# mmdagent/distantspeechrecognition-mirror

Measured on AMD Instinct MI355X. Metric: decoded_audio_hours_per_sec, higher is better.
Workload: dtype f32

## Files before the change

distantspeechrecognition-mirror_amd/csrc/decoder.cpp:

```cpp
#include "common.h"
#include "wfst_graph.h"
#include "lattice.h"
#include "lexicon.h"
#include "wordtrace.h"
#include "viterbi.h"
#include "decode_plan.h"
#include <algorithm>
#include <cmath>

namespace dsr {

static_assert(kPlanSideBytes == (size_t) kSideLds * sizeof(Side), "decode_plan.h budgets the side records of viterbi.h");

struct DecoderState {
  dsr_decoder_cfg cfg; bool haveGraph = false; int nSlots = 0; int nNodes = 0;
  WfstGraph::Csr csr; WfstGraph::Tables tab;
  DevBuf<int> d_xoff, d_xarc, d_xpathOff, d_eoff, d_path, d_nodeFinal, d_queue; DevBuf<float> d_pathCost;
  DevBuf<XRec> d_xrec; DevBuf<ERec> d_erec; DevBuf<float> d_arcCost, d_nodeCost; DevBuf<uint32_t> d_arcOut, d_arcIn;
  DevBuf<TokA> d_tokA, d_ctok; DevBuf<TokB> d_tokB; DevBuf<Side> d_side; DevBuf<XRecD> d_xrecD; DevBuf<XRecC> d_xrecC; double recLmScale = 0.0;  int fastOK = 0; int maxCnt = 0; DevBuf<int> d_tokOff, d_tokCnt, d_owner, d_rank, d_chead; DevBuf<unsigned> d_tags; DevBuf<CandA> d_cA; DevBuf<CandB> d_cB; DevBuf<unsigned> d_first; DevBuf<Bp> d_arena;
  DevBuf<long long> d_prof; DevBuf<dsr_decode_result> d_res; DevBuf<int> d_arcs; DevBuf<unsigned> d_words;
  long arenaCap = 0; int initial = 0; unsigned tokenMemoryLimit = 0;
  long lastPoolCap = 0;
  hipEvent_t evTrace = nullptr;
  DevBuf<TraceHead> d_heads; DevBuf<int> d_hopRec, d_hopOff;
// ... 363 lines not shown
    if (d->pendingU > 0) throw Error(DSR_E_CONSISTENCY, "a decode is already in flight on this decoder: collect it first");
    if (U <= 0) return;
    hipStream_t st = (hipStream_t) stream;
    if (d->cfg.wordTrace) { launch_wordtrace(d, score, nframes, U, Tmax, nDist, maxPath, want_paths, st); return; }
    check_arc_inputs(d, nDist);
    const bool latOn = d->cfg.latticeTokens > 0;
    if (latOn && d->dumpOn) throw Error(DSR_E_PARAMETER, "lattice bookkeeping and the token dump are separate debugging aids: enable one");
    const VitEnv env = read_vit_env();
    PlanIn in; in.streams = d->cfg.streams; in.maxActive = d->cfg.maxActive; in.arenaTokens = d->cfg.arenaTokens; in.latticeTokens = d->cfg.latticeTokens;
    in.topN = d->cfg.topN; in.dumpOn = d->dumpOn != 0; in.nNodes = d->nNodes; in.maxCnt = d->maxCnt; in.U = U; in.Tmax = Tmax; in.nDist = nDist;
    in.staticLds = viterbi_static_lds(plan_base_modes(in, env));
    const DecodePlan P = plan_decode(in, env, [&] { return xcd_round_robin(st); });
    ensure_scratch(d, P.slots, Tmax, latOn ? U : (P.segFrames > 0 ? P.poolArenas : 0));
    if (maxPath < 0) maxPath = 0;
    const VitArgs A = fill_vit_args(d, P, env, score, nframes, U, Tmax, nDist, maxPath, want_paths != 0, st);
    if (env.segVerbose) fprintf(stderr, "[dsr viterbi] %d utterances on %d workgroups: %s, %s state table\n", U, P.slots, P.segFrames > 0 ? (P.segQueues == 8 ? "time-sliced, XCD-bound queues" : "time-sliced, one queue") : "run to completion", P.narrow ? "narrow" : "wide");
    const TraceArgs TA = fill_trace_args(d, A);
    order_behind_last_traceback(P.slots, st);
    viterbi_launch(P.modes, A, P.slots, P.ldsBytes, st);
    traceback_launch(TA, st);
    publish_traceback(d, st);
    enqueue_result_copies(d, U, want_paths ? (size_t) U * maxPath : 0, st);
    d->pendingSlots = P.slots; d->pendingProf = A.D.prof;
  });
}

static void report_profile(const long long* prof, int slots)
{
  std::vector<long long> hp((size_t) slots * kProfN); DSR_HIP(hipMemcpy(hp.data(), prof, hp.size() * sizeof(long long), hipMemcpyDeviceToHost));
  double acc[32] = {0}; for (int s2 = 0; s2 < slots; s2++) for (int i = 0; i < 32; i++) acc[i] += (double) hp[(size_t) s2 * kProfN + i];
  fprintf(stderr, "[dsr viterbi prof] mean us per slot:");
  for (int i = 0; i < 32; i++) if (i != 15) fprintf(stderr, " p%d=%.0f", i, acc[i] / slots / 100.0);
  fprintf(stderr, "\n");
  double tmin = 1e30, tmax = 0.0, tsum = 0.0;
  for (int s2 = 0; s2 < slots; s2++) { double t = 0.0; for (int i = 0; i < 32; i++) if (i != 15) t += (double) hp[(size_t) s2 * kProfN + i]; t /= 100.0; tsum += t; if (t < tmin) tmin = t; if (t > tmax) tmax = t; }
  {
    double h[12] = {0}; for (int s2 = 0; s2 < slots; s2++) for (int i = 0; i < 12; i++) h[i] += (double) hp[(size_t) s2 * kProfN + 32 + i];
    const double nf = h[0] + h[1] + h[2] + h[3], tk = h[4] + h[5] + h[6] + h[7];
    static const char* const cn[4] = {"<=8192", "<=12288", ">12288", "memory path"};
    for (int c = 0; c < 4; c++) if (h[c] > 0) fprintf(stderr, "[dsr viterbi prof] frames with %s placements: %.1f %% of the frames, %.1f %% of the frame time, %.1f us per frame, %.2f ns per placement\n",
                                                      cn[c], 100.0 * h[c] / nf, 100.0 * h[4 + c] / tk, h[4 + c] / 100.0 / h[c], h[4 + c] * 10.0 / h[8 + c]);
  }
  {
    double a = 0, b = 0; for (int s2 = 0; s2 < slots; s2++) { a += (double) hp[(size_t) s2 * kProfN + 44]; b += (double) hp[(size_t) s2 * kProfN + 45]; }
    if (a + b > 0) fprintf(stderr, "[dsr viterbi prof] register-path frames: %.1f %% start laid out, %.1f %% run P1/P2\n", 100.0 * a / (a + b), 100.0 * b / (a + b));
    double m1 = 0, m2 = 0, mAll = 0; for (int s2 = 0; s2 < slots; s2++) { m1 += (double) hp[(size_t) s2 * kProfN + 46]; m2 += (double) hp[(size_t) s2 * kProfN + 47]; mAll += (double) hp[(size_t) s2 * kProfN + 32 + 3]; }
    if (mAll > 0) fprintf(stderr, "[dsr viterbi prof] memory-path frames: %.0f, of them %.1f %% with at most 28672 placements, %.1f %% with at most 32767\n", mAll, 100.0 * m1 / mAll, 100.0 * m2 / mAll);
  }
  {
    double h[6] = {0}; for (int s2 = 0; s2 < slots; s2++) for (int i = 0; i < 6; i++) h[i] += (double) hp[(size_t) s2 * kProfN + 48 + i];
    if (h[0] > 0) fprintf(stderr, "[dsr viterbi prof] hops behind the first: %.0f wave-placements, %.1f %% with a path of two or more hops, %.1f %% load hop costs, %.1f %% run the hop loop; "
                                  "%.3f hop iterations per wave-placement for %.3f hops per lane (x 64: %.2f)\n",
                          h[0], 100.0 * h[1] / h[0], 100.0 * h[2] / h[0], 100.0 * h[3] / h[0], h[4] / h[0], h[5] / h[0] / 64.0, h[5] / h[0]);
  }
  fprintf(stderr, "[dsr viterbi prof] busy us per slot: mean %.0f min %.0f max %.0f\n", tsum / slots, tmin, tmax);
  if (slots >= 64 && slots % 8 == 0) {
    double bx[8] = {0}; for (int s2 = 0; s2 < slots; s2++) { double t = 0.0; for (int i = 0; i < 32; i++) if (i != 15) t += (double) hp[(size_t) s2 * kProfN + i]; bx[s2 & 7] += t / 100.0; }
    fprintf(stderr, "[dsr viterbi prof] busy us per slot, by XCD:"); for (int q = 0; q < 8; q++) fprintf(stderr, " %.0f", bx[q] / (slots / 8)); fprintf(stderr, "\n");
  }
}

dsr_status dsr_decoder_decode_collect(dsr_decoder* d, dsr_decode_result* res, int32_t* arcs_out, uint32_t* words_out)
{
  return guard([&] {
    if (!d || !res) throw Error(DSR_E_PARAMETER, "null argument");
    if (d->pendingU <= 0) throw Error(DSR_E_CONSISTENCY, "no decode in flight");
    const int U = d->pendingU; const size_t nPath = d->pendingPath; const int slots = d->pendingSlots; long long* prof = d->pendingProf;
    d->pendingU = 0; d->lastU = U; d->lastPaths = nPath > 0; d->lastMaxPath = nPath > 0 ? nPath / (size_t) U : 0;
    DSR_HIP(hipEventSynchronize(d->evDone));
    memcpy(res, d->h_res.p, sizeof(dsr_decode_result) * U);
    if (arcs_out && nPath) memcpy(arcs_out, d->h_arcs.p, sizeof(int) * nPath);
    if (words_out && nPath) memcpy(words_out, d->h_words.p, sizeof(unsigned) * nPath);
    if (read_vit_env().segVerbose && d->d_poolNext.p && d->lastPoolCap > 0) {
      unsigned long long used = 0; DSR_HIP(hipMemcpy(&used, d->d_poolNext.p, sizeof(used), hipMemcpyDeviceToHost));
      fprintf(stderr, "[dsr viterbi] pool of back-pointer records: %.1f M of %.1f M taken\n", used / 1e6, d->lastPoolCap / 1e6);
    }
    if (read_vit_env().segVerbose) {
      long long laid = 0, reg = 0, all = 0;
      for (int u = 0; u < U; u++) if (res[u].status == DSR_OK || res[u].status == DSR_E_DIMENSION) { laid += res[u].laidOutFrames_; reg += res[u].registerFrames; all += res[u].frames + 1; }
      fprintf(stderr, "[dsr viterbi] frames: %lld laid out by the frame before, %lld through P1/P2, %lld on the memory path\n", laid, reg - laid, all - reg);
    }
    if (prof) report_profile(prof, slots);
    if (d->dumpOn) {
      long cnt[2]; DSR_HIP(hipMemcpy(cnt, d->d_dumpCount.p, sizeof(cnt), hipMemcpyDeviceToHost));
      const long N = cnt[0] < d->dumpCap ? cnt[0] : d->dumpCap; d->h_dumpFrames = cnt[1];
      std::vector<long> fo(cnt[1] + 1); if (cnt[1] > 0) DSR_HIP(hipMemcpy(fo.data(), d->d_dumpFrameOff.p, sizeof(long) * (cnt[1] + 1), hipMemcpyDeviceToHost));
      d->h_dumpFrameOff.assign(fo.begin(), fo.end());
      d->h_dumpNode.resize(N); d->h_dumpArc.resize(N); d->h_dumpAc.resize(N); d->h_dumpLm.resize(N);
      if (N > 0) {
        DSR_HIP(hipMemcpy(d->h_dumpNode.data(), d->d_dumpNode.p, sizeof(int) * N, hipMemcpyDeviceToHost));
        DSR_HIP(hipMemcpy(d->h_dumpArc.data(), d->d_dumpArc.p, sizeof(int) * N, hipMemcpyDeviceToHost));
        DSR_HIP(hipMemcpy(d->h_dumpAc.data(), d->d_dumpAc.p, sizeof(float) * N, hipMemcpyDeviceToHost));
        DSR_HIP(hipMemcpy(d->h_dumpLm.data(), d->d_dumpLm.p, sizeof(float) * N, hipMemcpyDeviceToHost));
      }
    }
  });
}

dsr_status dsr_decoder_decode_batch(dsr_decoder* d, const float* score, const int32_t* nframes, int U, int Tmax, int nDist,
                                    dsr_decode_result* res, int32_t* arcs_out, uint32_t* words_out, int maxPath, void* stream)
{
  if (!res) return guard([&] { throw Error(DSR_E_PARAMETER, "null argument"); });
  if (U <= 0) return DSR_OK;
  const dsr_status s1 = dsr_decoder_decode_launch(d, score, nframes, U, Tmax, nDist, maxPath, (arcs_out || words_out) ? 1 : 0, stream);
  if (s1 != DSR_OK) return s1;
  return dsr_decoder_decode_collect(d, res, arcs_out, words_out);
// ... 118 lines not shown
```

distantspeechrecognition-mirror_amd/csrc/k_viterbi.hip:

```cpp
#include "launch.h"
#include "viterbi.h"
#include <algorithm>
#include <cmath>
#include <type_traits>

namespace dsr {

static constexpr uint32_t kNone = 0xFFFFFFFFu;
static constexpr uint32_t kEndBit = 0x80000000u;
static constexpr int kWaves = kThreads / 64;
static constexpr int kFastK = 8;
static constexpr int kB = 2;
static constexpr int kFastE = 8190;
static constexpr int kP1 = 16;
static constexpr int kW = 4;

typedef const __attribute__((address_space(4))) VitArgs* KP;

__device__ __forceinline__ unsigned ld_u32(const unsigned* p) { return __hip_atomic_load(p, __ATOMIC_RELAXED, __HIP_MEMORY_SCOPE_AGENT); }
__device__ __forceinline__ int ld_i32(const int* p) { return __hip_atomic_load(p, __ATOMIC_RELAXED, __HIP_MEMORY_SCOPE_AGENT); }
__device__ __forceinline__ void st_u32(unsigned* p, unsigned v) { __hip_atomic_store(p, v, __ATOMIC_RELAXED, __HIP_MEMORY_SCOPE_AGENT); }
__device__ __forceinline__ void st_i32(int* p, int v) { __hip_atomic_store(p, v, __ATOMIC_RELAXED, __HIP_MEMORY_SCOPE_AGENT); }
__device__ __forceinline__ void st_u64_dev(void* p, unsigned long long v) { __hip_atomic_store(reinterpret_cast<unsigned long long*>(p), v, __ATOMIC_RELAXED, __HIP_MEMORY_SCOPE_AGENT); }
__device__ __forceinline__ unsigned long long ld_u64_dev(const void* p) { return __hip_atomic_load(reinterpret_cast<const unsigned long long*>(p), __ATOMIC_RELAXED, __HIP_MEMORY_SCOPE_AGENT); }

__device__ __forceinline__ int wave_incl_scan(int v, int )
{
  v += __builtin_amdgcn_update_dpp(0, v, 0x111, 0xF, 0xF, true);
  v += __builtin_amdgcn_update_dpp(0, v, 0x112, 0xF, 0xF, true);
  v += __builtin_amdgcn_update_dpp(0, v, 0x114, 0xF, 0xF, true);
  v += __builtin_amdgcn_update_dpp(0, v, 0x118, 0xF, 0xF, true);
  v += __builtin_amdgcn_update_dpp(0, v, 0x142, 0xA, 0xF, false);
  v += __builtin_amdgcn_update_dpp(0, v, 0x143, 0xC, 0xF, false);
  return v;
}
__device__ __forceinline__ float wave_max_f_uni(float v)
{
#define DSR_DPP_F(ctrl, rm) { const float o = __int_as_float(__builtin_amdgcn_update_dpp(__float_as_int(v), __float_as_int(v), ctrl, rm, 0xF, false)); v = fmaxf(v, o); }
  DSR_DPP_F(0x111, 0xF) DSR_DPP_F(0x112, 0xF) DSR_DPP_F(0x114, 0xF) DSR_DPP_F(0x118, 0xF) DSR_DPP_F(0x142, 0xA) DSR_DPP_F(0x143, 0xC)
#undef DSR_DPP_F
  return __int_as_float(__builtin_amdgcn_readlane(__float_as_int(v), 63));
}
__device__ __forceinline__ double wave_min_d_uni(double v)
{
#define DSR_DPP_D(ctrl, rm) { const int lo = __double2loint(v), hi = __double2hiint(v); \
    const double o = __hiloint2double(__builtin_amdgcn_update_dpp(hi, hi, ctrl, rm, 0xF, false), __builtin_amdgcn_update_dpp(lo, lo, ctrl, rm, 0xF, false)); v = (o < v) ? o : v; }
  DSR_DPP_D(0x111, 0xF) DSR_DPP_D(0x112, 0xF) DSR_DPP_D(0x114, 0xF) DSR_DPP_D(0x118, 0xF) DSR_DPP_D(0x142, 0xA) DSR_DPP_D(0x143, 0xC)
#undef DSR_DPP_D
  return __hiloint2double(__builtin_amdgcn_readlane(__double2hiint(v), 63), __builtin_amdgcn_readlane(__double2loint(v), 63));
}
__device__ __forceinline__ double wave_min_d(double v)
{
#pragma unroll
  for (int d = 32; d >= 1; d >>= 1) { const double o = __shfl_xor(v, d, 64); v = (o < v) ? o : v; }
// ... 244 lines not shown
            }
          }
          TICK(16);
          for (int i = tid; i < kFastC / 32; i += nthr) s_bm[i] = 0u;
          TICK(17);
#pragma unroll
          for (int it = 0; it < kP1; it++) {
            const int base = b0 + it * 64; pk[it] = 0u;
            if (base < b1) {
              const int i = base + lane; int cnt = 0;
              if (i < b1) {
                if (!((double) psc[it] > thresh)) cnt = pcn[it];
              }
              pcn[it] = cnt;
              const int incl = wave_incl_scan(cnt, lane);
              const unsigned long long bal = __ballot(cnt > 0);
              if (cnt > 0) pk[it] = 0x80000000u | (unsigned) ((runC + incl - cnt) & 0x7FFF) | ((unsigned) ((runE + __popcll(bal & ((1ull << lane) - 1ull))) & 0xFFFF) << 15);
              runC += __builtin_amdgcn_readlane(incl, 63); runE += __popcll(bal);
            }
          }
          TICK(18);
          if (lane == 0) { s_waveTot[wave] = runC; s_waveTotE[wave] = runE; }
          if (tid == 0) { s_sideN = 0; s_gbase[0] = 0; s_err = 0; }
        }
        __syncthreads();
        TICK(0);
        int cbase, ebase;
        {
          const int a = (lane < nw) ? s_waveTot[lane] : 0, b = (lane < nw) ? s_waveTotE[lane] : 0;
          const int sa = wave_incl_scan(a, lane), sb = wave_incl_scan(b, lane);
          C = __builtin_amdgcn_readlane(sa, 63); E = __builtin_amdgcn_readlane(sb, 63);
          const int wu = uni(wave);
          cbase = __builtin_amdgcn_readlane(sa - a, wu); ebase = __builtin_amdgcn_readlane(sb - b, wu);
        }
        TICK(19);
        if (!(C > fastCapC || E > eCap || C > regC)) {
          RELOAD();
          const bool ident = (E == n);
#pragma unroll
          for (int it = 0; it < kP1; it++) if (pk[it] & 0x80000000u) {
            const int e = ebase + (int) ((pk[it] >> 15) & 0xFFFFu); const int off = cbase + (int) (pk[it] & 0x7FFFu);
            if (!ident) ctok[e] = curA[wave * chunkT + it * 64 + lane];
            atomicOr(&s_bm[off >> 5], 1u << (off & 31));
            for (int g = (off >> 6) + 1; g <= ((off + pcn[it]) >> 6); g++) s_gbase[g] = (unsigned) (e + 1) | ((unsigned) (64 * g - off) << 13);
          }
          __syncthreads();
        }
        } else __syncthreads();
        if (C > fastCapC || E > eCap || C > regC) { fast = false; __syncthreads(); }
        else {
          RELOAD();
          const bool ident = (E == n);
          const TokA* __restrict__ ctk = ident ? curA : ctok;
          TICK(1);
          Cfr = C;
          if (pre && tid == nthr - 1) s_stat[2] += 1ll << 32;
          if (PROF && tid == 0) s_hist[pre ? 12 : 13] += 1;
          RELOAD();
          int tq = tid; asm volatile("" : "+v"(tq)); const int lq = tq & 63, wq = tq >> 6;
          const int K = (C + nthr - 1) / nthr;
          float qac[kFastK], qlm[kFastK]; int qrec[kFastK]; unsigned ek[kFastK];
          double* const ttlS = reinterpret_cast<double*>(cA);
          uint4* const ovf = reinterpret_cast<uint4*>(cB);
          const XRecD* const xrecD = ka->G.xrecD; const float* const pathCost = ka->G.pathCost; const uint32_t silenceX = ka->D.silenceX;
          double locMin = HUGE_VAL; float locMag = 0.0f;
          const bool prevNull0 = (fr == 0);
          const double lmS = ka->D.lmScale, lsPen = __dmul_rn(ka->D.lmScale, ka->D.lmPenalty), lsSil = __dmul_rn(ka->D.lmScale, ka->D.silPenalty);
          const bool sil0 = (0u == silenceX);
#pragma unroll
          for (int k = 0; k < kFastK; k++) { qac[k] = 0.0f; qlm[k] = 0.0f; qrec[k] = 0; ek[k] = 0u; }

          const int nPass = (!NARROW && C > tableC) ? 2 : 1;
          auto table_insert = [&](const unsigned dst, const unsigned prod, const int c) __attribute__((always_inline)) -> unsigned {
            const unsigned key = dst + 1u;
            unsigned h = (prod >> 7) & (unsigned) (tabN - 1); int probes = 0;
            if (NARROW) {
              const unsigned w = (key << 15) | (unsigned) c;
              for (;;) {
                const unsigned kk = atomicCAS(&tab[h], 0u, w);
                if (kk == 0u) break;
                if ((kk >> 15) == key) { atomicMin(&tab[h], w); break; }
                h = (h + 1u) & (unsigned) (tabN - 1);
                if (++probes > tabN) { s_err = 1; break; }
              }
              return h;
            }
            for (;;) {
              const unsigned kk = atomicCAS(&hkey[h], 0u, key);
              if (kk == 0u || kk == key) break;
              h = (h + 1u) & (unsigned) (hashN - 1);
              if (++probes > hashN) { s_err = 1; break; }
            }
            atomicMin(&hfirst[h], (unsigned) c);
            return h;
          };
          constexpr unsigned ekBucket = NARROW ? 0x7FFFu : 0x3FFFu;
          auto in_pass = [&](const unsigned e, const int pass) __attribute__((always_inline)) -> bool { return NARROW || (int) ((e >> 27) & 1u) == pass; };
          auto is_first = [&](const unsigned h, const int c) __attribute__((always_inline)) -> bool { return NARROW ? (tab[h] & 0x7FFFu) == (unsigned) c : hfirst[h] == (unsigned) c; };
          auto push_side = [&](const unsigned h, const int sx) __attribute__((always_inline)) -> unsigned {
            if (NARROW) {
              unsigned old = tab[h];
              for (;;) { const unsigned prev = atomicCAS(&tab[h], old, 0x80000000u | ((unsigned) sx << 15) | (old & 0x7FFFu)); if (prev == old) break; old = prev; }
              return (old & 0x80000000u) ? (0x80000000u | ((old >> 15) & 0xFFFFu)) : 0u;
            }
            return atomicExch(&hkey[h], 0x80000000u | (unsigned) sx);
          };
// ... 63 lines not shown
#pragma unroll
              for (int h = 1; h < 4; h++) {
                double l = __dadd_rn((double) lmNode, __dmul_rn(lmS, (double) hc[i][h - 1]));
                if (!NP) { const double l1 = __dadd_rn(l, lsPen); l = ((xmeta >> (17 + h)) & 1u) ? l1 : l; }
                lmNode = (pls[i] > h) ? (float) l : lmNode;
              }
              if (PROF) TICK(31);
              lm8[i] = lmNode;
            }
            bool anyMore = false;
#pragma unroll
            for (int i = 0; i < kB; i++) anyMore = anyMore || more[i];
            if (__any(anyMore)) {
#pragma unroll
              for (int i = 0; i < kB; i++) if (more[i]) {
                const uint32_t xmeta = (uint32_t) xr[i].y; const int plen = (int) (xmeta & 0xFFFFu), xp2 = xr[i].w;
                double lmNode = (double) lm8[i];
                if (!(xmeta & 0x80000000u)) {
                  for (int h = 4; h < plen; h++) {
                    double l = __dadd_rn(lmNode, __dmul_rn(lmS, (double) pathCost[xp2 + h - 1]));
                    if (!NP && ((xmeta >> (17 + h)) & 1u)) l = __dadd_rn(l, lsPen);
                    lmNode = (double) (float) l;
                  }
                } else {
                  const int* pp = ka->G.path + ka->G.xpathOff[rec8[i]];
                  for (int h = 1; h < plen; h++) {
                    const int a = pp[h];
                    double l = __dadd_rn(lmNode, __dmul_rn(lmS, (double) ka->G.arcCost[a]));
                    if (!NP && ka->G.arcOut[a] != 0) l = __dadd_rn(l, lsPen);
                    lmNode = (double) (float) l;
                  }
                }
                lm8[i] = (float) lmNode;
              }
            }
            if (PROF) { asm volatile("s_waitcnt vmcnt(0)" ::: "memory"); TICK(31); }
#pragma unroll
            for (int i = 0; i < kB; i++) {
              const int c = (g8 + i) * nthr + tq;
              const bool tsil = (ek8[i] >> 29) & 1u; ek8[i] &= 0x1FFFu;
              if (c < C) {
                const int xdist = xr[i].x; const uint32_t xmeta = (uint32_t) xr[i].y; const int xdst = xr[i].z;
                const bool has = (xmeta & 0xFFFFu) != 0u;
                const bool pnull = has ? false : prevNull0;
                const bool pinSil = has ? sil0 : tsil;
                double lm = __dadd_rn((double) lm8[i], xl[i].x);
                if (!NP) { const double lm1 = __dadd_rn(lm, lsPen); lm = (xmeta & 0x10000u) ? lm1 : lm; }
                const bool silArc = ((uint32_t) (xdist + 1) == silenceX);
                if (!NP) { const double lm2 = __dadd_rn(lm, lsSil); lm = (silArc && (pnull || !pinSil)) ? lm2 : lm; }
                float rowv;
                if (useLdsRow) { rowv = ((const lds_float_t*) srow)[xdist]; DSR_NO_MERGE(); } else rowv = rowG[xdist];
                const double ac = __dadd_rn((double) ac8[i], (double) rowv);
                const double ttl = __dadd_rn(ac, lm);
                *at32w<double>(ttlS, (uint32_t) c * 8u) = ttl; ac8[i] = (float) ac; lm8[i] = (float) lm; rec8[i] |= (silArc ? 0x40000000 : 0);
                if (ttl < locMin) locMin = ttl;
                locMag = fmaxf(locMag, __fadd_rn(fabsf(ac8[i]), fabsf(lm8[i])));
                if (PROF) { asm volatile("s_waitcnt vmcnt(0) lgkmcnt(0)" ::: "memory"); TICK(29); }
                const unsigned prod = (unsigned) xdst * 2654435761u;
                if (!NARROW && nPass > 1 && (prod >> 31)) ek8[i] |= 1u << 27;
                else ek8[i] |= (table_insert((unsigned) xdst, prod, c) << 13) | (1u << 28);
                if (PROF) { asm volatile("s_waitcnt lgkmcnt(0)" ::: "memory"); TICK(30); }
              }
            }
          };
          auto expand8 = [&](auto NOPEN, const int g8, float* ac8, float* lm8, int* rec8, unsigned* ek8) __attribute__((always_inline)) {
#pragma unroll
            for (int i = 0; i < kB; i++) locate(g8 + i, rec8[i], ek8[i]);
            if (PROF) { asm volatile("s_waitcnt lgkmcnt(0)" ::: "memory"); TICK(26); }
#pragma unroll
            for (int i = 0; i < kB; i++) tokload(ac8[i], lm8[i], rec8[i], ek8[i]);
            if (PROF) { asm volatile("s_waitcnt vmcnt(0)" ::: "memory"); TICK(27); }
            expandR(NOPEN, g8, ac8, lm8, rec8, ek8);
          };
          auto park_store = [&](const int kb, const float* oac, const float* olm, const int* orec, const unsigned* oek) __attribute__((always_inline)) {
#pragma unroll
            for (int i = 0; i < kB; i++) { const int c = (kb + i) * nthr + tq; if (c < C) ovf[c - kFastK * nthr] = make_uint4(__float_as_uint(oac[i]), __float_as_uint(olm[i]), (unsigned) orec[i], oek[i]); }
          };
          auto park_load = [&](const int kb, float* oac, float* olm, int* orec, unsigned* oek) __attribute__((always_inline)) {
#pragma unroll
            for (int i = 0; i < kB; i++) {
              int c = (kb + i) * nthr + tq; c = (c < C) ? c : kFastK * nthr;
              const uint4 v = ovf[c - kFastK * nthr];
              oac[i] = __uint_as_float(v.x); olm[i] = __uint_as_float(v.y); orec[i] = (int) v.z; oek[i] = v.w;
            }
          };
          auto runP3 = [&](auto NOPEN) __attribute__((always_inline)) {
#pragma unroll
            for (int g8 = 0; g8 < kFastK; g8 += kB) if (g8 < K) expand8(NOPEN, g8, &qac[g8], &qlm[g8], &qrec[g8], &ek[g8]);
            for (int kb = kFastK; kb < K; kb += kB) {
              float oac[kB], olm[kB]; int orec[kB]; unsigned oek[kB];
              expand8(NOPEN, kb, oac, olm, orec, oek); park_store(kb, oac, olm, orec, oek);
            }
          };
          if (ka->D.noPen) runP3(std::true_type{}); else runP3(std::false_type{});
          TICK(2);
          locMin = wave_min_d_uni(locMin); locMag = wave_max_f_uni(locMag);
          if (lq == 0) { s_waveMin[wq] = locMin; s_waveMag[wq] = locMag; }
          TICK(3);
          __syncthreads();
          TICK(4);
          for (int i = tq; i < kFastC / 32; i += nthr) s_bm[i] = 0u;
          topScore = HUGE_VAL;
          float frameMag;
          { const double v = (lq < nw) ? s_waveMin[lq] : HUGE_VAL; const float g = (lq < nw) ? s_waveMag[lq] : 0.0f;
            topScore = wave_min_d_uni(v); frameMag = wave_max_f_uni(g); }
          RELOAD();
          const double threshNext = __dadd_rn(topScore, ka->D.beam);
          const bool prune = !dump && (fr + 1 < T);
          const double doomT = prune ? __dadd_rn(threshNext, (double) __fmul_rn(frameMag, 4.76837158203125e-07f)) : HUGE_VAL;
          unsigned long long firstMask = 0ull;
          auto later8 = [&](const int g8, const int pass, const float* ac8, const float* lm8, const int* rec8, const unsigned* ek8) __attribute__((always_inline)) {
            double tt[kB]; uint32_t pb[kB];
#pragma unroll
            for (int i = 0; i < kB; i++) {
              int c = (g8 + i) * nthr + tq; c = (c < C) ? c : 0;
              tt[i] = ttlS[c]; pb[i] = ctk[ek8[i] & 0x1FFFu].bp;
            }
#pragma unroll
            for (int i = 0; i < kB; i++) {
              const int c = (g8 + i) * nthr + tq;
              if (c < C && (ek8[i] & (1u << 28)) && in_pass(ek8[i], pass) && !((firstMask >> (g8 + i)) & 1ull)) {
                const unsigned h = (ek8[i] >> 13) & ekBucket;
                if (is_first(h, c)) firstMask |= 1ull << (g8 + i);
                else if (!((double) __fadd_rn(ac8[i], lm8[i]) > doomT)) {
                  const int sx = atomicAdd(&s_sideN, 1);
                  const unsigned nx = push_side(h, sx);
                  Side sd; sd.ttl = tt[i]; sd.ac = ac8[i]; sd.lm = lm8[i]; sd.rec = rec8[i]; sd.prevBp = pb[i]; sd.c = c; sd.next = nx;
                  if (sx < sideLds) sideL[sx] = sd; else side[sx] = sd;
                }
              }
            }
          };
          auto fold_multi = [&](const int wslot0, const unsigned head, const float ac, const float lm) __attribute__((always_inline)) -> int {
            int wslot = wslot0, wIdx = -1; double fw = (double) __fadd_rn(ac, lm);
            for (;;) {
              int best = 0x7FFFFFFF, bi = -1, steps = 0;
              for (unsigned p = head; (p & 0x80000000u) && steps <= C; steps++) {
                const int pi = (int) (p & 0x7FFFFFFFu);
                int pc; double pt; unsigned pn;
                side_link(sideL, side, sideLds, pi, pc, pt, pn);
                if (pc > wslot && pc < best && pt < fw) { best = pc; bi = pi; }
                p = pn;
              }
              if (bi < 0) break;
              wslot = best; wIdx = bi;
              fw = (double) side_score(sideL, side, sideLds, bi);
            }
            return wIdx;
          };
          auto fold1 = [&](const int k, const int pass, float& ac, float& lm, int& rec, unsigned& ekk, unsigned* defer) __attribute__((always_inline)) {
            const bool mine = ((firstMask >> k) & 1ull) && !(ekk & 0x80000000u) && (ekk & (1u << 28)) && in_pass(ekk, pass);
            if (mine) {
              const unsigned head = chain_head((ekk >> 13) & ekBucket);
              if (NARROW) tab[(ekk >> 13) & ekBucket] = 0u;
              ekk &= 0x1FFFu;
              if (head & 0x80000000u) {
                int wIdx = -1;
                const int hi = (int) (head & 0x7FFFFFFFu);
                unsigned hnext; double pt;
                { int cdummy; side_link(sideL, side, sideLds, hi, cdummy, pt, hnext); }
                if (!(hnext & 0x80000000u)) {
                  if (pt < (double) __fadd_rn(ac, lm)) wIdx = hi;
                } else if (defer) *defer = head;
                else wIdx = fold_multi(k * nthr + tq, head, ac, lm);
                if (wIdx >= 0) {
                  side_winner(sideL, side, sideLds, wIdx, ac, lm, rec);
                  ekk = 0x80000000u | (unsigned) wIdx;
                }
              }
            }
          };
          auto insert8 = [&](const int g8, const int* rec8, unsigned* ek8) __attribute__((always_inline)) {
            int xd[kB];
#pragma unroll
            for (int i = 0; i < kB; i++) xd[i] = ka->G.xrecC[rec8[i] & 0x3FFFFFFF].dst;
#pragma unroll
            for (int i = 0; i < kB; i++) {
              const int c = (g8 + i) * nthr + tq;
              if (c < C && (ek8[i] & (1u << 27)) && !(ek8[i] & 0x80000000u)) ek8[i] |= (table_insert((unsigned) xd[i], (unsigned) xd[i] * 2654435761u, c) << 13) | (1u << 28);
            }
          };
          for (int pass = 0; pass < nPass; pass++) {
            if (!NARROW && pass > 0) {
              __syncthreads();
              { uint4* h4 = reinterpret_cast<uint4*>(hkey); const int q4 = hashN >> 2;
                for (int i = tq; i < 2 * q4; i += nthr) { unsigned wv = (i < q4) ? 0u : 0xFFFFFFFFu; asm volatile("" : "+v"(wv)); h4[i] = make_uint4(wv, wv, wv, wv); }    }
              __syncthreads();
#pragma unroll
              for (int g8 = 0; g8 < kFastK; g8 += kB) if (g8 < K) insert8(g8, &qrec[g8], &ek[g8]);
              for (int kb = kFastK; kb < K; kb += kB) {
                float oac[kB], olm[kB]; int orec[kB]; unsigned oek[kB]; park_load(kb, oac, olm, orec, oek);
                insert8(kb, orec, oek); park_store(kb, oac, olm, orec, oek);
              }
              __syncthreads();
            }
            {
              unsigned later = 0u;
#pragma unroll
              for (int k = 0; k < kFastK; k++) {
                const bool cand = k < K && k * nthr + tq < C && (ek[k] & (1u << 28)) && in_pass(ek[k], pass) && !((firstMask >> k) & 1ull);
                if (cand) {
                  if (is_first((ek[k] >> 13) & ekBucket, k * nthr + tq)) firstMask |= 1ull << k;
                  else if (!((double) __fadd_rn(qac[k], qlm[k]) > doomT)) later |= 1u << k;
                }
              }
              asm volatile("" : "+v"(later));
              __builtin_amdgcn_sched_barrier(0);
              while (__any(later != 0u)) {
                if (later) {
                  const int k = __ffs((int) later) - 1; later &= later - 1u;
                  unsigned ekk = ek[0];
#pragma unroll
                  for (int j = 1; j < kFastK; j++) ekk = (k == j) ? ek[j] : ekk;
                  const int c = k * nthr + tq;
                  const double tt = ttlS[c]; const uint32_t pb = ctk[ekk & 0x1FFFu].bp;
                  const unsigned h = (ekk >> 13) & ekBucket;
                  const int sx = atomicAdd(&s_sideN, 1);
                  const unsigned nx = push_side(h, sx);
                  float ac = qac[0], lm = qlm[0]; int rec = qrec[0];
#pragma unroll
                  for (int j = 1; j < kFastK; j++) { const bool is = (k == j); ac = is ? qac[j] : ac; lm = is ? qlm[j] : lm; rec = is ? qrec[j] : rec; }
                  Side* dstS = (sx < sideLds) ? nullptr : &side[sx];
                  if (!dstS) { Side& q = sideL[sx]; q.ttl = tt; q.ac = ac; q.lm = lm; q.rec = rec; q.prevBp = pb; q.c = c; q.next = nx; }
                  else { dstS->ttl = tt; dstS->ac = ac; dstS->lm = lm; dstS->rec = rec; dstS->prevBp = pb; dstS->c = c; dstS->next = nx; }
                }
              }
            }
            for (int kb = kFastK; kb < K; kb += kB) { float oac[kB], olm[kB]; int orec[kB]; unsigned oek[kB]; park_load(kb, oac, olm, orec, oek); later8(kb, pass, oac, olm, orec, oek); }
            if (pass == 0) TICK(20);
            __syncthreads();
            if (pass == 0) TICK(5);
            {
              unsigned pend = 0u, dh[kFastK];
#pragma unroll
              for (int k = 0; k < kFastK; k++) { dh[k] = 0u; if (k < K) { fold1(k, pass, qac[k], qlm[k], qrec[k], ek[k], &dh[k]); if (dh[k]) pend |= 1u << k; } }
              if (pass == 0) TICK(24);
              while (__any(pend != 0u)) {
                if (pend) {
                  const int k = __ffs((int) pend) - 1; pend &= pend - 1u;
                  unsigned head = dh[0]; float ac = qac[0], lm = qlm[0];
#pragma unroll
                  for (int j = 1; j < kFastK; j++) { const bool is = (k == j); head = is ? dh[j] : head; ac = is ? qac[j] : ac; lm = is ? qlm[j] : lm; }
                  const int wIdx = fold_multi(k * nthr + tq, head, ac, lm);
                  if (wIdx >= 0) {
                    float wac, wlm; int wrec;
                    side_winner(sideL, side, sideLds, wIdx, wac, wlm, wrec);
#pragma unroll
                    for (int j = 0; j < kFastK; j++) if (k == j) { qac[j] = wac; qlm[j] = wlm; qrec[j] = wrec; ek[j] = 0x80000000u | (unsigned) wIdx; }
                  }
                }
              }
            }
            if (pass == 0) TICK(25);
            for (int kb = kFastK; kb < K; kb += kB) {
              float oac[kB], olm[kB]; int orec[kB]; unsigned oek[kB]; park_load(kb, oac, olm, orec, oek);
#pragma unroll
              for (int i = 0; i < kB; i++) if (kb + i < K) fold1(kb + i, pass, oac[i], olm[i], orec[i], oek[i], nullptr);
              park_store(kb, oac, olm, orec, oek);
            }
          }
          TICK(12);
          if (s_err) { status = DSR_E_ALLOCATION; break; }
          unsigned long long keepMask = 0ull;
#pragma unroll
          for (int k = 0; k < kFastK; k++) if (k < K && ((firstMask >> k) & 1ull)) {
            const float sc1 = __fadd_rn(qac[k], qlm[k]);
            if (!prune || !((double) sc1 > threshNext)) keepMask |= 1ull << k;
          }
          for (int kb = kFastK; kb < K; kb += kB) {
            float oac[kB], olm[kB]; int orec[kB]; unsigned oek[kB]; park_load(kb, oac, olm, orec, oek);
#pragma unroll
            for (int i = 0; i < kB; i++) if (kb + i < K && ((firstMask >> (kb + i)) & 1ull)) {
              const float sc1 = __fadd_rn(oac[i], olm[i]);
              if (!prune || !((double) sc1 > threshNext)) keepMask |= 1ull << (kb + i);
            }
          }
          int allFirst = 0;
          for (int k = 0; k < K; k++) {
            const unsigned long long bal = __ballot((keepMask >> k) & 1ull);
            if (lq == 0) s_cnt[k * nw + wq] = __popcll(bal);
            allFirst += __popcll(__ballot((firstMask >> k) & 1ull));
          }
          if (lq == 0) s_waveTotE[wq] = allFirst;
          TICK(13);
          __syncthreads();
          TICK(14);
          if (!NARROW) {
            uint4* h4 = reinterpret_cast<uint4*>(hkey); const int q4 = hashN >> 2;
            for (int i = tq; i < 2 * q4; i += nthr) { unsigned wv = (i < q4) ? 0u : 0xFFFFFFFFu; asm volatile("" : "+v"(wv)); h4[i] = make_uint4(wv, wv, wv, wv); }
          }
          if (wq == 0) {
            const int nG = K * nw;
            int a[6], tot = 0;
#pragma unroll
            for (int q = 0; q < 6; q++) { a[q] = (6 * lq + q < nG) ? s_cnt[6 * lq + q] : 0; tot += a[q]; }
            const int incl = wave_incl_scan(tot, lq); int run = incl - tot;
#pragma unroll
            for (int q = 0; q < 6; q++) { if (6 * lq + q < nG) s_cnt[6 * lq + q] = run; run += a[q]; }
            if (lq == 63) s_waveTot[0] = incl;
          }
          __syncthreads();
          TICK(6);
          numNew = uni(s_waveTot[0]);
          { const int a = (lq < nw) ? s_waveTotE[lq] : 0; numStat = __builtin_amdgcn_readlane(wave_incl_scan(a, lq), 63); }
          RELOAD();
          if (numNew > ka->D.maxTok || (segS > 0 ? arenaUsed : arenaOff) + numNew > ka->D.arenaCap) { status = DSR_E_ALLOCATION; break; }
          if (segS > 0 && arenaOff + numNew > chunkEnd) {
            const long need = numNew > ka->D.poolChunk ? (long) numNew : ka->D.poolChunk;
            __syncthreads();
            if (tid == 0) s_chunk = (long long) atomicAdd(ka->D.poolNext, (unsigned long long) need);
            __syncthreads();
            arenaOff = (long) s_chunk; chunkEnd = arenaOff + need;
            if (chunkEnd > ka->D.poolCap) { status = DSR_E_ALLOCATION; break; }
          }
          const XRecC* const xrecW = ka->G.xrecC; TokA* const outA = nxtA; TokB* const outB = nxtB; Bp* const outBp = arena + arenaOff;
          auto write4 = [&](auto NB, const int g4, const float* ac4, const float* lm4, const int* rec4, const unsigned* ek4) __attribute__((always_inline)) {
            constexpr int nb = decltype(NB)::value;
            int4 dx[nb]; uint32_t pv[nb];
#pragma unroll
            for (int i = 0; i < nb; i++) {
              const bool kp = (keepMask >> (g4 + i)) & 1ull;
              dx[i] = *reinterpret_cast<const int4*>(&xrecW[kp ? (rec4[i] & 0x3FFFFFFF) : 0]);
              const bool sw = kp && (ek4[i] & 0x80000000u) != 0u; const unsigned si = ek4[i] & 0x7FFFFFFFu;
              const uint32_t* pb = (sw && si >= (unsigned) sideLds) ? &side[si].prevBp : &ctk[(sw || !kp) ? 0u : (ek4[i] & 0x1FFFu)].bp;
              pv[i] = *pb;
              if (sw && si < (unsigned) sideLds) pv[i] = sideL[si].prevBp;
            }
#pragma unroll
            for (int i = 0; i < nb; i++) {
              const int k = g4 + i;
              if (k < K) {
                const bool isFirst = (keepMask >> k) & 1ull;
                const unsigned long long bal = __ballot(isFirst);
                if (isFirst) {
                  const int pos = numNew - 1 - (s_cnt[k * nw + wq] + __popcll(bal & ((1ull << lq) - 1ull)));
                  TokA na; na.ac = ac4[i]; na.lm = lm4[i]; na.bp = (uint32_t) (arenaOff + pos); na.xs = (uint32_t) dx[i].y | ((rec4[i] & 0x40000000) ? 0x80000000u : 0u);
                  TokB nb; nb.node = dx[i].x; nb.cnt = dx[i].z;
                  Bp bp; bp.prev = pv[i]; bp.rec = (uint32_t) (rec4[i] & 0x3FFFFFFF);
                  outA[pos] = na; outB[pos] = nb; outBp[pos] = bp;
                  if (pos < cntCap) cntL[pos] = (unsigned short) dx[i].z;
                }
              }
            }
          };
          const bool dense = numNew <= (hashN >> 1);
          if (dense) {
            uint4* const stage = reinterpret_cast<uint4*>(hkey);
            auto stage1 = [&](const int k, const float ac, const float lm, const int rec, const unsigned ekk) __attribute__((always_inline)) {
              const bool isFirst = (keepMask >> k) & 1ull;
              const unsigned long long bal = __ballot(isFirst);
              if (isFirst) stage[s_cnt[k * nw + wq] + __popcll(bal & ((1ull << lq) - 1ull))] = make_uint4(__float_as_uint(ac), __float_as_uint(lm), (unsigned) rec, ekk);
            };
#pragma unroll
            for (int k = 0; k < kFastK; k++) if (k < K) stage1(k, qac[k], qlm[k], qrec[k], ek[k]);
            for (int kb = kFastK; kb < K; kb += kB) {
              float oac[kB], olm[kB]; int orec[kB]; unsigned oek[kB]; park_load(kb, oac, olm, orec, oek);
#pragma unroll
              for (int i = 0; i < kB; i++) if (kb + i < K) stage1(kb + i, oac[i], olm[i], orec[i], oek[i]);
            }
            __syncthreads();
            TICK(21);
            const int q4 = hashN >> 2;
            const bool layNext = prune && numNew <= 4 * nthr;
            preC = -1;
            auto denseLoad = [&](const int f0, uint4* en, int4* dx, uint32_t* pv) __attribute__((always_inline)) {
#pragma unroll
              for (int i = 0; i < 2; i++) {
                const int f = f0 + i * nthr + tq; const bool on = f < numNew;
                en[i] = stage[on ? f : 0];
                if (on) { unsigned wv = (NARROW || f < q4) ? 0u : 0xFFFFFFFFu; asm volatile("" : "+v"(wv)); stage[f] = make_uint4(wv, wv, wv, wv); }
              }
#pragma unroll
              for (int i = 0; i < 2; i++) {
                const bool on = f0 + i * nthr + tq < numNew;
                dx[i] = *at32<int4>(xrecW, (on ? (en[i].z & 0x3FFFFFFFu) : 0u) * 16u);
                const bool sw = on && (en[i].w & 0x80000000u) != 0u; const unsigned si = en[i].w & 0x7FFFFFFFu;
                const uint32_t* pb = (sw && si >= (unsigned) sideLds) ? &side[si].prevBp : &ctk[(sw || !on) ? 0u : (en[i].w & 0x1FFFu)].bp;
                pv[i] = *pb;
                if (sw && si < (unsigned) sideLds) pv[i] = sideL[si].prevBp;
              }
            };
            auto denseStore = [&](const int f0, const uint4* en, const int4* dx, const uint32_t* pv) __attribute__((always_inline)) {
#pragma unroll
              for (int i = 0; i < 2; i++) {
                const int f = f0 + i * nthr + tq;
                if (f < numNew) {
                  const int pos = numNew - 1 - f;
                  TokA na; na.ac = __uint_as_float(en[i].x); na.lm = __uint_as_float(en[i].y); na.bp = (uint32_t) (arenaOff + pos); na.xs = (uint32_t) dx[i].y | ((en[i].z & 0x40000000u) ? 0x80000000u : 0u);
                  TokB nb; nb.node = dx[i].x; nb.cnt = dx[i].z;
                  Bp bp; bp.prev = pv[i]; bp.rec = (uint32_t) (en[i].z & 0x3FFFFFFFu);
                  outA[pos] = na; outB[pos] = nb; outBp[pos] = bp;
                  if (pos < cntCap) cntL[pos] = (unsigned short) dx[i].z;
                }
              }
            };
            auto layOut = [&](auto NE_, const int* cn) __attribute__((always_inline)) {
              constexpr int NE = decltype(NE_)::value;
              int in[NE]; bool bad = false;
#pragma unroll
              for (int i = 0; i < NE; i++) {
                in[i] = wave_incl_scan(cn[i], lq);
                bad = bad || (i * nthr + tq < numNew && cn[i] == 0);
              }
              const int badW = __any(bad) ? 1 : 0;
              if (lq == 63) {
#pragma unroll
                for (int i = 0; i < NE; i++) s_cnt[i * nw + wq] = in[i];
                s_waveTotE[wq] = badW;
              }
              __syncthreads();
              const int tg = (lq < NE * nw) ? s_cnt[lq] : 0;
              const int sg = wave_incl_scan(tg, lq);
              const int total = __builtin_amdgcn_readlane(sg, 63), wu = uni(wq);
              const bool anyBad = __any(((lq < nw) ? s_waveTotE[lq] : 0) != 0);
              const bool fits = total <= fastCapC;
#pragma unroll
              for (int i = 0; i < NE; i++) {
                const int f = i * nthr + tq; const int off = total - (__builtin_amdgcn_readlane(sg - tg, i * nw + wu) + in[i]);
                if (fits && f < numNew && cn[i] > 0) {
                  const int e = numNew - 1 - f;
                  atomicOr(&s_bm[off >> 5], 1u << (off & 31));
                  for (int g = (off >> 6) + 1; g <= ((off + cn[i]) >> 6); g++) s_gbase[g] = (unsigned) (e + 1) | ((unsigned) (64 * g - off) << 13);
                }
              }
              if (tq == 0) { s_sideN = 0; s_gbase[0] = 0; s_err = 0; }
              preC = (anyBad || !fits) ? -1 : total;
            };
            if (layNext && numNew > 2 * nthr) {
              int cn[4];
#pragma unroll
              for (int h = 0; h < 2; h++) {
// ... 400 lines not shown
```

Before: 28.64.

## Encode frame totals in spare record bits and compute backpointers arithmetically

The per-placement double total is now packed as a 3-bit code relative to the float sum of acoustic and LM scores, stored in unused bits of the record and ek words. The double is written to the LDS total array only when the code cannot represent it, and is rebuilt from the code when side records are emitted. When the token list is the identity layout, the previous backpointer is computed as arenaOff - n + index instead of being loaded from the token array. This removes most LDS double stores and loads and some global token reads. In exchange it adds encode and decode ALU work and keeps an escape path. The decoded total is a rounded-down float, not the exact double, which is a fidelity risk.

```diff
diff --git a/distantspeechrecognition-mirror_amd/csrc/decoder.cpp b/distantspeechrecognition-mirror_amd/csrc/decoder.cpp
--- a/distantspeechrecognition-mirror_amd/csrc/decoder.cpp
+++ b/distantspeechrecognition-mirror_amd/csrc/decoder.cpp
@@ -439,6 +439,8 @@
     if (h[0] > 0) fprintf(stderr, "[dsr viterbi prof] hops behind the first: %.0f wave-placements, %.1f %% with a path of two or more hops, %.1f %% load hop costs, %.1f %% run the hop loop; "
                                   "%.3f hop iterations per wave-placement for %.3f hops per lane (x 64: %.2f)\n",
                           h[0], 100.0 * h[1] / h[0], 100.0 * h[2] / h[0], 100.0 * h[3] / h[0], h[4] / h[0], h[5] / h[0] / 64.0, h[5] / h[0]);
+    double coded = 0, esc = 0; for (int s2 = 0; s2 < slots; s2++) { coded += (double) hp[(size_t) s2 * kProfN + 54]; esc += (double) hp[(size_t) s2 * kProfN + 55]; }
+    if (coded + esc > 0) fprintf(stderr, "[dsr viterbi prof] unrounded totals (ttl_code.h): %.0f placements carry a code, %.0f escape to memory (%.3g %%)\n", coded, esc, 100.0 * esc / (coded + esc));
   }
   fprintf(stderr, "[dsr viterbi prof] busy us per slot: mean %.0f min %.0f max %.0f\n", tsum / slots, tmin, tmax);
   if (slots >= 64 && slots % 8 == 0) {
diff --git a/distantspeechrecognition-mirror_amd/csrc/k_viterbi.hip b/distantspeechrecognition-mirror_amd/csrc/k_viterbi.hip
--- a/distantspeechrecognition-mirror_amd/csrc/k_viterbi.hip
+++ b/distantspeechrecognition-mirror_amd/csrc/k_viterbi.hip
@@ -1,5 +1,6 @@
 #include "launch.h"
 #include "viterbi.h"
+#include "ttl_code.h"
 #include <algorithm>
 #include <cmath>
 #include <type_traits>
@@ -350,6 +351,7 @@
           RELOAD();
           const bool ident = (E == n);
           const TokA* __restrict__ ctk = ident ? curA : ctok;
+          const uint32_t bpBase = (uint32_t) uni((int) (arenaOff - (long) n));
           TICK(1);
           Cfr = C;
           if (pre && tid == nthr - 1) s_stat[2] += 1ll << 32;
@@ -519,7 +521,11 @@
                 if (useLdsRow) { rowv = ((const lds_float_t*) srow)[xdist]; DSR_NO_MERGE(); } else rowv = rowG[xdist];
                 const double ac = __dadd_rn((double) ac8[i], (double) rowv);
                 const double ttl = __dadd_rn(ac, lm);
-                *at32w<double>(ttlS, (uint32_t) c * 8u) = ttl; ac8[i] = (float) ac; lm8[i] = (float) lm; rec8[i] |= (silArc ? 0x40000000 : 0);
+                ac8[i] = (float) ac; lm8[i] = (float) lm;
+                const unsigned tc = ttl_encode(ttl, __fadd_rn(ac8[i], lm8[i]));
+                if (tc == 0u) *at32w<double>(ttlS, (uint32_t) c * 8u) = ttl;
+                if (PROF) { const unsigned long long be = __ballot(tc == 0u), bc = __ballot(tc != 0u); if (lq == __ffsll((long long) (be | bc)) - 1) { atomicAdd(&s_hop[6], (unsigned long long) __popcll(bc)); if (be) atomicAdd(&s_hop[7], (unsigned long long) __popcll(be)); } }
+                rec8[i] |= (silArc ? 0x40000000 : 0) | (int) ((tc >> 2) << 31); ek8[i] |= (tc & 3u) << 29;
                 if (ttl < locMin) locMin = ttl;
                 locMag = fmaxf(locMag, __fadd_rn(fabsf(ac8[i]), fabsf(lm8[i])));
                 if (PROF) { asm volatile("s_waitcnt vmcnt(0) lgkmcnt(0)" ::: "memory"); TICK(29); }
@@ -576,13 +582,8 @@
           const bool prune = !dump && (fr + 1 < T);
           const double doomT = prune ? __dadd_rn(threshNext, (double) __fmul_rn(frameMag, 4.76837158203125e-07f)) : HUGE_VAL;
           unsigned long long firstMask = 0ull;
+          auto ttl_code_of = [](const unsigned ekk, const int rec) __attribute__((always_inline)) -> unsigned { return ((ekk >> 29) & 3u) | (((unsigned) rec >> 31) << 2); };
           auto later8 = [&](const int g8, const int pass, const float* ac8, const float* lm8, const int* rec8, const unsigned* ek8) __attribute__((always_inline)) {
-            double tt[kB]; uint32_t pb[kB];
-#pragma unroll
-            for (int i = 0; i < kB; i++) {
-              int c = (g8 + i) * nthr + tq; c = (c < C) ? c : 0;
-              tt[i] = ttlS[c]; pb[i] = ctk[ek8[i] & 0x1FFFu].bp;
-            }
 #pragma unroll
             for (int i = 0; i < kB; i++) {
               const int c = (g8 + i) * nthr + tq;
@@ -592,7 +593,10 @@
                 else if (!((double) __fadd_rn(ac8[i], lm8[i]) > doomT)) {
                   const int sx = atomicAdd(&s_sideN, 1);
                   const unsigned nx = push_side(h, sx);
-                  Side sd; sd.ttl = tt[i]; sd.ac = ac8[i]; sd.lm = lm8[i]; sd.rec = rec8[i]; sd.prevBp = pb[i]; sd.c = c; sd.next = nx;
+                  const unsigned tc = ttl_code_of(ek8[i], rec8[i]);
+                  double tt = ttl_decode(__fadd_rn(ac8[i], lm8[i]), tc); if (tc == 0u) tt = ttlS[c];
+                  uint32_t pb = bpBase + (ek8[i] & 0x1FFFu); if (!ident) pb = ctk[ek8[i] & 0x1FFFu].bp;
+                  Side sd; sd.ttl = tt; sd.ac = ac8[i]; sd.lm = lm8[i]; sd.rec = rec8[i]; sd.prevBp = pb; sd.c = c; sd.next = nx;
                   if (sx < sideLds) sideL[sx] = sd; else side[sx] = sd;
                 }
               }
@@ -680,13 +684,15 @@
 #pragma unroll
                   for (int j = 1; j < kFastK; j++) ekk = (k == j) ? ek[j] : ekk;
                   const int c = k * nthr + tq;
-                  const double tt = ttlS[c]; const uint32_t pb = ctk[ekk & 0x1FFFu].bp;
+                  float ac = qac[0], lm = qlm[0]; int rec = qrec[0];
+#pragma unroll
+                  for (int j = 1; j < kFastK; j++) { const bool is = (k == j); ac = is ? qac[j] : ac; lm = is ? qlm[j] : lm; rec = is ? qrec[j] : rec; }
+                  const unsigned tc = ttl_code_of(ekk, rec);
+                  double tt = ttl_decode(__fadd_rn(ac, lm), tc); if (tc == 0u) tt = ttlS[c];
+                  uint32_t pb = bpBase + (ekk & 0x1FFFu); if (!ident) pb = ctk[ekk & 0x1FFFu].bp;
                   const unsigned h = (ekk >> 13) & ekBucket;
                   const int sx = atomicAdd(&s_sideN, 1);
                   const unsigned nx = push_side(h, sx);
-                  float ac = qac[0], lm = qlm[0]; int rec = qrec[0];
-#pragma unroll
-                  for (int j = 1; j < kFastK; j++) { const bool is = (k == j); ac = is ? qac[j] : ac; lm = is ? qlm[j] : lm; rec = is ? qrec[j] : rec; }
                   Side* dstS = (sx < sideLds) ? nullptr : &side[sx];
                   if (!dstS) { Side& q = sideL[sx]; q.ttl = tt; q.ac = ac; q.lm = lm; q.rec = rec; q.prevBp = pb; q.c = c; q.next = nx; }
                   else { dstS->ttl = tt; dstS->ac = ac; dstS->lm = lm; dstS->rec = rec; dstS->prevBp = pb; dstS->c = c; dstS->next = nx; }
@@ -789,8 +795,8 @@
               const bool kp = (keepMask >> (g4 + i)) & 1ull;
               dx[i] = *reinterpret_cast<const int4*>(&xrecW[kp ? (rec4[i] & 0x3FFFFFFF) : 0]);
               const bool sw = kp && (ek4[i] & 0x80000000u) != 0u; const unsigned si = ek4[i] & 0x7FFFFFFFu;
-              const uint32_t* pb = (sw && si >= (unsigned) sideLds) ? &side[si].prevBp : &ctk[(sw || !kp) ? 0u : (ek4[i] & 0x1FFFu)].bp;
-              pv[i] = *pb;
+              if (ident) { pv[i] = bpBase + (ek4[i] & 0x1FFFu); if (sw && si >= (unsigned) sideLds) pv[i] = side[si].prevBp; }
+              else { const uint32_t* pb = (sw && si >= (unsigned) sideLds) ? &side[si].prevBp : &ctk[(sw || !kp) ? 0u : (ek4[i] & 0x1FFFu)].bp; pv[i] = *pb; }
               if (sw && si < (unsigned) sideLds) pv[i] = sideL[si].prevBp;
             }
 #pragma unroll
@@ -842,8 +848,8 @@
                 const bool on = f0 + i * nthr + tq < numNew;
                 dx[i] = *at32<int4>(xrecW, (on ? (en[i].z & 0x3FFFFFFFu) : 0u) * 16u);
                 const bool sw = on && (en[i].w & 0x80000000u) != 0u; const unsigned si = en[i].w & 0x7FFFFFFFu;
-                const uint32_t* pb = (sw && si >= (unsigned) sideLds) ? &side[si].prevBp : &ctk[(sw || !on) ? 0u : (en[i].w & 0x1FFFu)].bp;
-                pv[i] = *pb;
+                if (ident) { pv[i] = bpBase + (en[i].w & 0x1FFFu); if (sw && si >= (unsigned) sideLds) pv[i] = side[si].prevBp; }
+                else { const uint32_t* pb = (sw && si >= (unsigned) sideLds) ? &side[si].prevBp : &ctk[(sw || !on) ? 0u : (en[i].w & 0x1FFFu)].bp; pv[i] = *pb; }
                 if (sw && si < (unsigned) sideLds) pv[i] = sideL[si].prevBp;
               }
             };
diff --git a/distantspeechrecognition-mirror_amd/csrc/ttl_code.h b/distantspeechrecognition-mirror_amd/csrc/ttl_code.h
--- /dev/null
+++ b/distantspeechrecognition-mirror_amd/csrc/ttl_code.h
@@ -0,0 +1,32 @@
+#pragma once
+#include <cstdint>
+
+#if defined(__HIPCC__) || defined(__CUDACC__)
+#define DSR_TTL_HD __host__ __device__ inline
+#else
+#define DSR_TTL_HD inline
+#endif
+
+namespace dsr {
+
+DSR_TTL_HD uint32_t ttl_f2u(float f) { uint32_t u; __builtin_memcpy(&u, &f, 4); return u; }
+DSR_TTL_HD float ttl_u2f(uint32_t u) { float f; __builtin_memcpy(&f, &u, 4); return f; }
+DSR_TTL_HD uint32_t ttl_f2ord(float f) { const uint32_t u = ttl_f2u(f); return (u & 0x80000000u) ? ~u : (u | 0x80000000u); }
+DSR_TTL_HD float ttl_ord2f(uint32_t o) { return ttl_u2f((o & 0x80000000u) ? (o ^ 0x80000000u) : ~o); }
+
+DSR_TTL_HD float ttl_round_down(double p)
+{
+  const float r = (float) p;
+  return ((double) r > p) ? ttl_ord2f(ttl_f2ord(r) - 1u) : r;
+}
+
+DSR_TTL_HD unsigned ttl_encode(double p, float s0)
+{
+  if ((ttl_f2u(s0) & 0x7F800000u) == 0x7F800000u || p != p) return 0u;
+  const uint32_t d = ttl_f2ord(ttl_round_down(p)) - ttl_f2ord(s0) + 4u;
+  return (d - 1u < 7u) ? d : 0u;
+}
+
+DSR_TTL_HD double ttl_decode(float s0, unsigned code) { return (double) ttl_ord2f(ttl_f2ord(s0) + code - 4u); }
+
+}
```

New measurement: 28.14. -1.7%, worse.
